# gMedAI-Lab/GAViKO

Hardware: AMD Instinct MI355X
Metric: MRI volumes/sec (fwd+bwd) ViT-B/16 gaviko, 120x160x160 (higher is better)
Workload: dtype bf16

## Files before the change

### gaviko_amd/csrc/gemm8p_bf16.hip

```cpp
#include "gemm_epilogue.hpp"

namespace gvk {

namespace {
constexpr int kUnit = 128 * 128;
constexpr int kBuf = 4 * kUnit;
constexpr int kLds = 2 * kBuf;

#define GVK_VMCNT(n) __builtin_amdgcn_s_waitcnt(0x0F70 | ((n) & 0xF) | (((n) >> 4) << 14))
#define GVK_LGKMCNT0() __builtin_amdgcn_s_waitcnt(0xC07F)

#ifdef GVK_STAMPS
#define GVK_STAMP(k) st_[k] = __builtin_amdgcn_s_memtime();
#ifndef GVK_ABLATE
#define GVK_ABLATE 0
#endif
#else
#define GVK_STAMP(k)
#define GVK_ABLATE 0
#endif
}

template <int EPI, int VAR>
__global__ __launch_bounds__(512) void gemm8p_kernel(GemmArgs p) {
  constexpr int BM = 256, BN = 256, BK = 64;
  extern __shared__ __attribute__((aligned(16))) char smem[];

  const int nwg = p.nbm * p.nbn;
  int wg;
  {
    const int bid = blockIdx.x, xcd = bid & 7, q = nwg >> 3, r = nwg & 7;
    wg = (xcd < r ? xcd * (q + 1) : r * (q + 1) + (xcd - r) * q) + (bid >> 3);
  }
  constexpr int GROUP_M = 8;
  const int gsz = GROUP_M * p.nbn;
  const int grp = wg / gsz, first_m = grp * GROUP_M;
  const int gm = min(p.nbm - first_m, GROUP_M);
  const int rem = wg - grp * gsz;
  const int tile_m = first_m + rem % gm, tile_n = rem / gm;
  const int m0 = tile_m * BM, n0 = tile_n * BN;

  const int lane = lane_id();
  const int wave = wave_id();
  const int wr = wave >> 2, wc = wave & 3;
#ifdef GVK_STAMPS
  unsigned long long st_[32];
#pragma unroll
  for (int k = 0; k < 32; ++k) st_[k] = 0;
  GVK_STAMP(0)
  const unsigned long long rt0_ = __builtin_amdgcn_s_memrealtime();
#endif
  const int l15 = lane & 15, lq = lane >> 4;

  const bf16* __restrict__ Ag = p.A + (size_t)m0 * p.lda;
  const bf16* __restrict__ Wg = p.W + (size_t)n0 * p.ldw;
  int aoff[2][2], woff[2][2];
#pragma unroll
  for (int r = 0; r < 2; ++r) {
    const int lr = (r * 8 + wave) * 8 + (lane >> 3), slot = lane & 7;
#pragma unroll
    for (int h = 0; h < 2; ++h) {
      const int mrow = min(128 * (lr >> 6) + 64 * h + (lr & 63), p.a_rows - 1 - m0);
      aoff[h][r] = mrow * p.lda + ((slot ^ swz_a128(lr)) << 3);
      const int nrow = 64 * (lr >> 5) + 32 * h + (lr & 31);
      woff[h][r] = nrow * p.ldw + ((slot ^ swz_w(lr)) << 3);
    }
  }
#define GVK_STAGE(U, T)                                                                                      \
  {                                                                                                          \
    const int t_ = (T);                                                                                      \
    char* dst_ = smem + (t_ & 1) * kBuf + (U) * kUnit + wave * 1024;                                         \
    const int k0_ = t_ * BK;                                                                                 \
    if constexpr ((U) == 0 || (U) == 2) {                                                                    \
      glds16(Wg + woff[(U) >> 1][0] + k0_, dst_);                                                            \
      glds16(Wg + woff[(U) >> 1][1] + k0_, dst_ + 8192);                                                     \
    } else {                                                                                                 \
      glds16(Ag + aoff[(U) >> 1][0] + k0_, dst_);                                                            \
      glds16(Ag + aoff[(U) >> 1][1] + k0_, dst_ + 8192);                                                     \
    }                                                                                                        \
  }

#define GVK_STAGE_HALF(U, T, R)                                                                              \
  if constexpr ((GVK_ABLATE & 1) == 0) {                                                                     \
    const int t_ = (T);                                                                                      \
    char* dst_ = smem + (t_ & 1) * kBuf + (U) * kUnit + wave * 1024 + (R) * 8192;                            \
    if constexpr ((U) == 0 || (U) == 2) glds16(Wg + woff[(U) >> 1][R] + t_ * BK, dst_);                      \
    else glds16(Ag + aoff[(U) >> 1][R] + t_ * BK, dst_);                                                     \
  }

  int ra[2], rw[2];
  {
    const int arow = 64 * wr + l15, wrow = 32 * wc + 8 * (l15 >> 2) + (l15 & 3);
#pragma unroll
    for (int ks = 0; ks < 2; ++ks) {
      ra[ks] = arow * 128 + (((4 * ks + lq) ^ swz_a128(arow)) << 4);
      rw[ks] = wrow * 128 + (((4 * ks + lq) ^ swz_w(wrow)) << 4);
    }
  }
  bf16x8 xa[4][2], w0[2][2], w1[2][2];
#define GVK_READ_A(MQ, BASE)                                                                                 \
  if constexpr ((GVK_ABLATE & 4) == 0)                                                                       \
  _Pragma("unroll") for (int i = 0; i < 4; ++i)                                                              \
  _Pragma("unroll") for (int ks = 0; ks < 2; ++ks)                                                           \
      xa[i][ks] = *(const bf16x8*)((BASE) + ((MQ) ? 3 : 1) * kUnit + ra[ks] + i * 2048);
#define GVK_READ_W(NQ, WREG, BASE)                                                                           \
  if constexpr ((GVK_ABLATE & 4) == 0)                                                                       \
  _Pragma("unroll") for (int j = 0; j < 2; ++j)                                                              \
  _Pragma("unroll") for (int ks = 0; ks < 2; ++ks)                                                           \
      WREG[j][ks] = *(const bf16x8*)((BASE) + ((NQ) ? 2 : 0) * kUnit + rw[ks] + j * 512);

  f32x4 acc[8][4];
#pragma unroll
  for (int i = 0; i < 8; ++i)
#pragma unroll
    for (int j = 0; j < 4; ++j) acc[i][j] = f32x4{0.f, 0.f, 0.f, 0.f};
#define GVK_MMA4(MQ, NQ, WREG, C_)                                                                           \
  if constexpr ((GVK_ABLATE & 2) == 0)                                                                       \
  _Pragma("unroll") for (int i = 2 * ((C_) & 1); i < 2 * ((C_) & 1) + 2; ++i)                                \
  _Pragma("unroll") for (int j = 0; j < 2; ++j)                                                              \
      acc[4 * (MQ) + i][2 * (NQ) + j] =                                                                      \
          __builtin_amdgcn_mfma_f32_16x16x32_bf16(WREG[j][(C_) >> 1], xa[i][(C_) >> 1], acc[4 * (MQ) + i][2 * (NQ) + j], 0, 0, 0);

#define GVK_COMPUTE(MQ, NQ, WREG, DO_STAGE, SU, ST_, SB)                                                     \
  __builtin_amdgcn_sched_barrier(0);                                                                         \
  __builtin_amdgcn_s_barrier();                                                                              \
  if constexpr ((SB) >= 0) { GVK_STAMP((SB) < 0 ? 0 : (SB)) }                                                \
  GVK_LGKMCNT0();                                                                                            \
  if constexpr ((SB) >= 0) { GVK_STAMP((SB) < 0 ? 0 : (SB) + 1) }                                            \
  __builtin_amdgcn_sched_barrier(0);                                                                         \
  __builtin_amdgcn_s_setprio(1);                                                                             \
  GVK_MMA4(MQ, NQ, WREG, 0)                                                                                  \
  if constexpr (VAR == 1 && (DO_STAGE)) {                                                                    \
    __builtin_amdgcn_sched_barrier(0);                                                                       \
    GVK_STAGE_HALF(SU, ST_, 0)                                                                               \
    __builtin_amdgcn_sched_barrier(0);                                                                       \
  }                                                                                                          \
  GVK_MMA4(MQ, NQ, WREG, 1)                                                                                  \
  GVK_MMA4(MQ, NQ, WREG, 2)                                                                                  \
  if constexpr (VAR == 1 && (DO_STAGE)) {                                                                    \
    __builtin_amdgcn_sched_barrier(0);                                                                       \
    GVK_STAGE_HALF(SU, ST_, 1)                                                                               \
    __builtin_amdgcn_sched_barrier(0);                                                                       \
  }                                                                                                          \
  GVK_MMA4(MQ, NQ, WREG, 3)                                                                                  \
  __builtin_amdgcn_s_setprio(0);                                                                             \
  __builtin_amdgcn_sched_barrier(0);                                                                         \
  if constexpr ((SB) >= 0) { GVK_STAMP((SB) < 0 ? 0 : (SB) + 2) }                                            \
  __builtin_amdgcn_s_barrier();                                                                              \
  if constexpr ((SB) >= 0) { GVK_STAMP((SB) < 0 ? 0 : (SB) + 3) }                                            \
  __builtin_amdgcn_sched_barrier(0);

#define GVK_KTILE(T, ST, VM0, VM1, VM3, SB)                                                                      \
  {                                                                                                          \
    const int tt_ = (T);                                                                                     \
    const char* base_ = smem + (tt_ & 1) * kBuf;                                                             \
    GVK_READ_W(0, w0, base_)                                                                                 \
    GVK_READ_A(0, base_)                                                                                     \
    if constexpr (VAR == 0 && ((ST) & 1) != 0 && (GVK_ABLATE & 1) == 0) GVK_STAGE(2, tt_ + 1)                                         \
    GVK_VMCNT(VM0);                                                                                          \
    GVK_COMPUTE(0, 0, w0, ((ST) & 1) != 0, 3, tt_ + 1, SB)                                                       \
    GVK_READ_W(1, w1, base_)                                                                                 \
    if constexpr (VAR == 0 && ((ST) & 2) != 0 && (GVK_ABLATE & 1) == 0) GVK_STAGE(3, tt_ + 1)                                         \
    GVK_VMCNT(VM1);                                                                                          \
    GVK_COMPUTE(0, 1, w1, ((ST) & 2) != 0, 0, tt_ + 2, (SB) < 0 ? -1 : (SB) + 4)                                                       \
    GVK_READ_A(1, base_)                                                                                     \
    if constexpr (VAR == 0 && ((ST) & 4) != 0 && (GVK_ABLATE & 1) == 0) GVK_STAGE(0, tt_ + 2)                                         \
    GVK_COMPUTE(1, 1, w1, ((ST) & 4) != 0, 1, tt_ + 2, (SB) < 0 ? -1 : (SB) + 8)                                                       \
    if constexpr (VAR == 0 && ((ST) & 8) != 0 && (GVK_ABLATE & 1) == 0) GVK_STAGE(1, tt_ + 2)                                         \
    GVK_VMCNT(VM3);                                                                                          \
    GVK_COMPUTE(1, 0, w0, ((ST) & 8) != 0, 2, tt_ + 2, (SB) < 0 ? -1 : (SB) + 12)                                                       \
  }

  const int nt = p.K / BK;
  GVK_STAGE(0, 0) GVK_STAGE(1, 0) GVK_STAGE(2, 0) GVK_STAGE(3, 0)
  GVK_STAGE(0, 1) GVK_STAGE(1, 1)
  if constexpr (VAR == 1) {
    GVK_STAGE(2, 1)
    GVK_VMCNT(10);
  } else {
    GVK_VMCNT(8);
  }
  __builtin_amdgcn_s_barrier();
  if (wr == 1) __builtin_amdgcn_s_barrier();
  __builtin_amdgcn_sched_barrier(0);
  GVK_STAMP(1)
  int t = 0;
#ifdef GVK_STAMPS
  for (; t < nt - 3; ++t) GVK_KTILE(t, 15, 8, 8, 8, -1)
  GVK_STAMP(2)
  if (nt >= 3) { GVK_KTILE(t, 15, 8, 8, 8, 4) ++t; }
  GVK_STAMP(20)
#else
  for (; t < nt - 2; ++t) GVK_KTILE(t, 15, 8, 8, 8, -1)
#endif
  if constexpr (VAR == 1) {
    GVK_KTILE(t, 1, 8, 8, 4, -1)
    ++t;
    GVK_KTILE(t, 0, 2, 0, 63, -1)
  } else {
    GVK_KTILE(t, 3, 8, 8, 4, -1)
    ++t;
    GVK_KTILE(t, 0, 2, 0, 63, -1)
  }
  if (wr == 0) __builtin_amdgcn_s_barrier();
#undef GVK_KTILE
#undef GVK_COMPUTE
#undef GVK_MMA4
#undef GVK_STAGE_HALF
#undef GVK_READ_A
#undef GVK_READ_W
#undef GVK_STAGE

  GVK_STAMP(21)
#ifdef GVK_STAMPS
  if constexpr ((GVK_ABLATE & 2) != 0) {
#pragma unroll
    for (int i = 0; i < 4; ++i) { asm volatile("" ::"v"(xa[i][0]), "v"(xa[i][1])); }
    asm volatile("" ::"v"(w0[0][0]), "v"(w0[1][1]), "v"(w1[0][0]), "v"(w1[1][1]));
  }
  const bf16* aux_keep = p.aux;
  p.aux = nullptr;
#endif
  gemm_epilogue<EPI, false, 8, 4>(p, acc, m0 + 128 * wr, n0 + 64 * wc, l15, lq);
#ifdef GVK_STAMPS
  __builtin_amdgcn_s_waitcnt(0x0F70);
  GVK_STAMP(22)
  st_[23] = rt0_;
  st_[24] = __builtin_amdgcn_s_memrealtime();
  if (aux_keep != nullptr && lane == 0) {
    unsigned long long* o = (unsigned long long*)aux_keep + ((size_t)blockIdx.x * 8 + wave) * 32;
#pragma unroll
    for (int k = 0; k < 32; ++k) o[k] = st_[k];
  }
#endif
}

template <int EPI, int VAR>
static int launch8p(const GemmArgs& a, hipStream_t stream) {
  static bool attr_set = false;
  if (!attr_set) {
    hipError_t e = hipFuncSetAttribute(reinterpret_cast<const void*>(&gemm8p_kernel<EPI, VAR>), hipFuncAttributeMaxDynamicSharedMemorySize, kLds);
    if (e != hipSuccess) return set_error(-3, "hipFuncSetAttribute(gemm8p): %s", hipGetErrorString(e));
    attr_set = true;
  }
  GemmArgs p = a;
  p.nbm = (a.M + 255) / 256;
  p.nbn = a.N / 256;
  p.a_rows = (a.M + 127) / 128 * 128;
  GVK_LAUNCH((gemm8p_kernel<EPI, VAR>), dim3(p.nbm * p.nbn), dim3(512), kLds, stream, p);
  return check_launch("gemm8p_bf16");
}

bool gemm8p_supports(int epilogue) {
  switch (epilogue) {
    case GVK_EPI_STORE_BF16: case GVK_EPI_BIAS_GELU_BF16: case GVK_EPI_GELU_BWD_BF16: case GVK_EPI_STORE_F32: case GVK_EPI_BIAS_RES_F32:
      return true;
    default:
      return false;
  }
}

template <int VAR>
static int launch8p_var(const GemmArgs& a, int epilogue, hipStream_t stream) {
  if (a.N % 256 != 0 || a.K % 64 != 0 || a.K < 128 || a.drop_thresh != 0u)
    return set_error(-2, "gemm8p: needs N %% 256 == 0, K %% 64 == 0, K >= 128 and no dropout (N=%d K=%d)", a.N, a.K);
  switch (epilogue) {
    case GVK_EPI_STORE_BF16: return launch8p<GVK_EPI_STORE_BF16, VAR>(a, stream);
    case GVK_EPI_BIAS_GELU_BF16: return launch8p<GVK_EPI_BIAS_GELU_BF16, VAR>(a, stream);
    case GVK_EPI_GELU_BWD_BF16: return launch8p<GVK_EPI_GELU_BWD_BF16, VAR>(a, stream);
    case GVK_EPI_STORE_F32: return launch8p<GVK_EPI_STORE_F32, VAR>(a, stream);
    case GVK_EPI_BIAS_RES_F32: return launch8p<GVK_EPI_BIAS_RES_F32, VAR>(a, stream);
    default: return set_error(-2, "gemm8p: epilogue %d is not built on the 256x256 eight-phase kernel", epilogue);
  }
}

int launch_gemm8p(const GemmArgs& a, int epilogue, int variant, hipStream_t stream) {
  return variant == 0 ? launch8p_var<0>(a, epilogue, stream) : launch8p_var<1>(a, epilogue, stream);
}

}
```

### gaviko_amd/csrc/gemm_bf16.hip

```cpp
#include "gemm_epilogue.hpp"

namespace gvk {

template <int BK>
__device__ __forceinline__ int swz_chunk(int row) {
  if constexpr (BK == 64) return (row >> 1) & 7;
  else return (0x78 >> (((row >> 2) & 3) * 2)) & 3;
}

template <int BM, int BN, int EPI, int BK = 64, bool DROP = false, int NS = 2, int NW = 4, bool SPLITK = false>
__global__ __launch_bounds__(64 * NW) void gemm_nt_kernel(GemmArgs p) {
  static_assert(NW == 4 || NW == 8, "4 or 8 waves");
  static_assert(!SPLITK || (NW == 4 && !DROP), "split-K is built on the 4-wave loops");
  static_assert(BK == 64, "the interleaved weight-row mapping is built for 128-byte tile rows");
  static_assert(NS >= 2 && NS <= 4, "2..4 LDS stages");
  constexpr int WM = BM / (NW / 2), WN = BN / 2;
  constexpr int MT = WM / 16, NT = WN / 16;
  constexpr int ROWB = BK * 2;
  constexpr int RPI = 1024 / ROWB;
  constexpr int CPR = ROWB / 16;
  constexpr int A_BYTES = BM * ROWB, W_BYTES = BN * ROWB, STAGE = A_BYTES + W_BYTES;
  extern __shared__ __attribute__((aligned(16))) char smem[];

  const int nwg = p.nbm * p.nbn;
  int wg;
  [[maybe_unused]] int piece = 0;
  if constexpr (SPLITK) {
    const int nu = nwg * p.ksplit;
    const int bid = blockIdx.x, xcd = bid & 7, q = nu >> 3, r = nu & 7;
    const int u = (xcd < r ? xcd * (q + 1) : r * (q + 1) + (xcd - r) * q) + (bid >> 3);
    wg = u / p.ksplit;
    piece = u - wg * p.ksplit;
  } else {
    const int bid = blockIdx.x, xcd = bid & 7, q = nwg >> 3, r = nwg & 7;
    wg = (xcd < r ? xcd * (q + 1) : r * (q + 1) + (xcd - r) * q) + (bid >> 3);
  }
  const int GROUP_M = p.group_m;
  const int gsz = GROUP_M * p.nbn;
  const int grp = wg / gsz, first_m = grp * GROUP_M;
  const int gm = min(p.nbm - first_m, GROUP_M);
  const int rem = wg - grp * gsz;
  int tile_m = first_m + rem % gm, tile_n = rem / gm;
  if (p.xcd_panels > 0) {
    tile_m = wg / p.nbn;
    tile_n = wg - tile_m * p.nbn;
  }
  const int m0 = tile_m * p.m_stride, n0 = tile_n * BN;

  const int lane = lane_id();
  const int wave = wave_id();
  const int wm = wave >> 1, wn = wave & 1;
  const int l15 = lane & 15, lq = lane >> 4;

  const bf16* __restrict__ Ag = p.A + (size_t)m0 * p.lda;
  const bf16* __restrict__ Wg = p.W + (size_t)n0 * p.ldw;
  if constexpr (SPLITK) {
    Ag += (size_t)piece * p.kt_per * BK;
    Wg += (size_t)piece * p.kt_per * BK;
  }

  auto stage = [&](int buf, int kt) {
    char* sA = smem + buf * STAGE;
    char* sW = sA + A_BYTES;
    const int k0 = kt * BK;
    const int rsub = lane / CPR, slot = lane % CPR;
#pragma unroll
    for (int r = 0; r < BM / (NW * RPI); ++r) {
      const int row = (r * NW + wave) * RPI + rsub;
      const int chunk = slot ^ swz_chunk<BK>(row);
      int srow = row;
      if constexpr (BM > 128 || 128 % BM != 0) srow = min(row, p.a_rows - 1 - m0);
      glds16(Ag + (size_t)srow * p.lda + k0 + chunk * 8, sA + (r * NW + wave) * 1024);
    }
#pragma unroll
    for (int r = 0; r < BN / (NW * RPI); ++r) {
      const int row = (r * NW + wave) * RPI + rsub;
      const int chunk = slot ^ swz_w(row);
      glds16(Wg + (size_t)row * p.ldw + k0 + chunk * 8, sW + (r * NW + wave) * 1024);
    }
  };

  f32x4 acc[MT][NT];
#pragma unroll
  for (int i = 0; i < MT; ++i)
#pragma unroll
    for (int j = 0; j < NT; ++j) acc[i][j] = f32x4{0.f, 0.f, 0.f, 0.f};

  int nt = p.K / BK;
  if constexpr (SPLITK) nt = min(p.kt_per, nt - piece * p.kt_per);
  if constexpr (BK == 64) {
#define GVK_LOAD_FRAGS(SA, SW, KS, XA, WB)                                                                  \
  {                                                                                                         \
    const int chunk_ = (KS) * 4 + lq;                                                                       \
    _Pragma("unroll") for (int i = 0; i < MT; ++i) {                                                        \
      const int row = wm * WM + i * 16 + l15;                                                               \
      XA[i] = *(const bf16x8*)((SA) + row * ROWB + ((chunk_ ^ swz_chunk<BK>(row)) << 4));                   \
    }                                                                                                       \
    _Pragma("unroll") for (int j = 0; j < NT; ++j) {                                                        \
      const int row = wn * WN + 32 * (j >> 1) + 8 * (l15 >> 2) + 4 * (j & 1) + (l15 & 3);                   \
      WB[j] = *(const bf16x8*)((SW) + row * ROWB + ((chunk_ ^ swz_w(row)) << 4));                           \
    }                                                                                                       \
  }
#define GVK_MMA(XA, WB)                                                                                      \
  _Pragma("unroll") for (int i = 0; i < MT; ++i)                                                            \
  _Pragma("unroll") for (int j = 0; j < NT; ++j)                                                            \
      acc[i][j] = __builtin_amdgcn_mfma_f32_16x16x32_bf16(WB[j], XA[i], acc[i][j], 0, 0, 0);
    bf16x8 xa0[MT], wb0[NT], xa1[MT], wb1[NT];
    constexpr int PER_TILE = BM / (NW * RPI) + BN / (NW * RPI);
    if constexpr (NS == 2) {
    stage(0, 0);
    if (nt > 1) stage(1, 1);
    if (nt > 1) __builtin_amdgcn_s_waitcnt(0x0F70 | (PER_TILE & 0xF) | ((PER_TILE >> 4) << 14));
    else __builtin_amdgcn_s_waitcnt(0x0F70);
    __builtin_amdgcn_s_barrier();
    GVK_LOAD_FRAGS(smem, smem + A_BYTES, 0, xa0, wb0)
    __builtin_amdgcn_s_waitcnt(0xC07F);
#define GVK_TILE(T, PREFETCH)                                                                               \
    {                                                                                                       \
      const int buf = (T) & 1;                                                                              \
      const char* sA = smem + buf * STAGE;                                                                  \
      const char* sW = sA + A_BYTES;                                                                        \
      GVK_LOAD_FRAGS(sA, sW, 1, xa1, wb1)                                                                   \
      __builtin_amdgcn_sched_barrier(0);                                                                    \
      GVK_MMA(xa0, wb0)                                                                                     \
      __builtin_amdgcn_sched_barrier(0);                                                                    \
      __syncthreads();     \
      if (PREFETCH) stage(buf, (T) + 2);                                                                    \
      GVK_LOAD_FRAGS(smem + (buf ^ 1) * STAGE, smem + (buf ^ 1) * STAGE + A_BYTES, 0, xa0, wb0)             \
      __builtin_amdgcn_sched_barrier(0);                                                                    \
      GVK_MMA(xa1, wb1)                                                                                     \
      __builtin_amdgcn_sched_barrier(0);                                                                    \
      __builtin_amdgcn_s_waitcnt(0xC07F);     \
    }
    int t = 0;
    for (; t < nt - 2; ++t) GVK_TILE(t, true)
    for (; t < nt; ++t) GVK_TILE(t, false)
#undef GVK_TILE
    } else {
    static_assert((NS - 1) * PER_TILE <= 63, "vmcnt is a 6-bit counter");
#pragma unroll
    for (int sgi = 0; sgi < NS; ++sgi)
      if (sgi < nt) stage(sgi, sgi);
    {
      const int ahead = min(nt, NS) - 1;
      if (ahead >= 3) __builtin_amdgcn_s_waitcnt(0x0F70 | ((3 * PER_TILE) & 0xF) | (((3 * PER_TILE) >> 4) << 14));
      else if (ahead == 2) __builtin_amdgcn_s_waitcnt(0x0F70 | ((2 * PER_TILE) & 0xF) | (((2 * PER_TILE) >> 4) << 14));
      else if (ahead == 1) __builtin_amdgcn_s_waitcnt(0x0F70 | (PER_TILE & 0xF) | ((PER_TILE >> 4) << 14));
      else __builtin_amdgcn_s_waitcnt(0x0F70);
    }
    __builtin_amdgcn_s_barrier();
    GVK_LOAD_FRAGS(smem, smem + A_BYTES, 0, xa0, wb0)
    __builtin_amdgcn_s_waitcnt(0xC07F);
#define GVK_TILE3(T, BUF, PREFETCH, AHEAD, LAST)                                                            \
    {                                                                                                       \
      const int buf = (BUF);                                                                                \
      const int nxt = buf == NS - 1 ? 0 : buf + 1;                                                          \
      const char* sA = smem + buf * STAGE;                                                                  \
      const char* sW = sA + A_BYTES;                                                                        \
      GVK_LOAD_FRAGS(sA, sW, 1, xa1, wb1)                                                                   \
      __builtin_amdgcn_sched_barrier(0);                                                                    \
      GVK_MMA(xa0, wb0)                                                                                     \
      __builtin_amdgcn_sched_barrier(0);                                                                    \
       \
      __builtin_amdgcn_s_waitcnt(0x0070 | (((AHEAD) * PER_TILE) & 0xF) | ((((AHEAD) * PER_TILE) >> 4) << 14)); \
      __builtin_amdgcn_s_barrier();                                                                         \
      if (PREFETCH) stage(buf, (T) + NS);                                                                   \
      if (!(LAST)) GVK_LOAD_FRAGS(smem + nxt * STAGE, smem + nxt * STAGE + A_BYTES, 0, xa0, wb0)            \
      __builtin_amdgcn_sched_barrier(0);                                                                    \
      GVK_MMA(xa1, wb1)                                                                                     \
      __builtin_amdgcn_sched_barrier(0);                                                                    \
      __builtin_amdgcn_s_waitcnt(0xC07F);                                                                   \
    }
    int t = 0, b = 0;
    for (; t < nt - NS; ++t) {
      GVK_TILE3(t, b, true, NS - 2, false)
      b = b == NS - 1 ? 0 : b + 1;
    }
    for (; t < nt; ++t) {
      const int r = nt - 1 - t;
      if (NS > 3 && r == 3) GVK_TILE3(t, b, false, 2, false)
      else if (r == 2) GVK_TILE3(t, b, false, 1, false)
      else if (r == 1) GVK_TILE3(t, b, false, 0, false)
      else GVK_TILE3(t, b, false, 0, true)
      b = b == NS - 1 ? 0 : b + 1;
    }
#undef GVK_TILE3
    }
#undef GVK_LOAD_FRAGS
#undef GVK_MMA
  }

  if constexpr (SPLITK) {
    const int tile_id = tile_m * p.nbn + tile_n;
    constexpr int kPiece = NW * MT * NT * 64 * 4;
    float* const base = p.sk_part + ((size_t)tile_id * p.ksplit) * kPiece;
    const __amdgpu_buffer_rsrc_t rs = __builtin_amdgcn_make_buffer_rsrc((void*)base, 0, p.ksplit * kPiece * 4, 0x00020000);
    const int off = ((wave * MT * NT) * 64 + lane) * 16;
#pragma unroll
    for (int i = 0; i < MT; ++i)
#pragma unroll
      for (int j = 0; j < NT; ++j)
        __builtin_amdgcn_raw_buffer_store_b128(__builtin_bit_cast(u32x4, acc[i][j]), rs, (piece * kPiece) * 4 + off + (i * NT + j) * 1024, 0, 16);
    int* const s_last = (int*)smem;
    asm volatile("s_waitcnt vmcnt(0)" ::: "memory");
    __syncthreads();
    if (threadIdx.x == 0) {
      const int t = __hip_atomic_fetch_add(p.sk_tick + tile_id, 1, __ATOMIC_RELAXED, __HIP_MEMORY_SCOPE_AGENT);
      const int last = (t == p.ksplit - 1) ? 1 : 0;
      if (last) {
        __builtin_amdgcn_fence(__ATOMIC_ACQUIRE, "agent");
        asm volatile("s_waitcnt vmcnt(0)" ::: "memory");
        __hip_atomic_store(p.sk_tick + tile_id, 0, __ATOMIC_RELAXED, __HIP_MEMORY_SCOPE_AGENT);
      }
      *s_last = last;
    }
    __syncthreads();
    if (!*s_last) return;
    if (p.ksplit == 2) {
      const int pc = piece ^ 1;
#pragma unroll
      for (int i = 0; i < MT; ++i)
#pragma unroll
        for (int j = 0; j < NT; ++j) acc[i][j] += *(const f32x4*)((const char*)base + (size_t)pc * kPiece * 4 + off + (i * NT + j) * 1024);
    } else {
#pragma unroll
      for (int i = 0; i < MT; ++i)
#pragma unroll
        for (int j = 0; j < NT; ++j) acc[i][j] = f32x4{0.f, 0.f, 0.f, 0.f};
      for (int pc = 0; pc < p.ksplit; ++pc) {
#pragma unroll
        for (int i = 0; i < MT; ++i)
#pragma unroll
          for (int j = 0; j < NT; ++j) acc[i][j] += *(const f32x4*)((const char*)base + (size_t)pc * kPiece * 4 + off + (i * NT + j) * 1024);
      }
    }
  }
  gemm_epilogue<EPI, DROP, MT, NT>(p, acc, m0 + wm * WM, n0 + wn * WN, l15, lq);
}

template <int BM, int BN, int EPI, bool DROP = false, int NS = 2, int NW = 4, bool SPLITK = false>
static int launch_gemm(const GemmArgs& a, hipStream_t stream) {
  constexpr int BK = 64;
  constexpr int lds = NS * (BM + BN) * BK * 2;
  static bool attr_set = false;
  if (!attr_set) {
    hipError_t e = hipFuncSetAttribute(reinterpret_cast<const void*>(&gemm_nt_kernel<BM, BN, EPI, BK, DROP, NS, NW, SPLITK>),
                                       hipFuncAttributeMaxDynamicSharedMemorySize, lds);
    if (e != hipSuccess) return set_error(-3, "hipFuncSetAttribute(gemm %dx%d): %s", BM, BN, hipGetErrorString(e));
    attr_set = true;
  }
  GemmArgs p = a;
  p.nbm = (a.M + BM - 1) / BM;
  p.nbn = a.N / BN;
  p.a_rows = (a.M + 127) / 128 * 128;
  p.m_stride = BM;
  if (a.m_stride > 0) {
    if (a.m_stride < BM || (long)(a.nbm - 1) * a.m_stride + BM > p.a_rows)
      return set_error(-2, "gvk_gemm_nt_bf16: %d row panels of %d rows at stride %d do not fit %d (padded) rows", a.nbm, BM, a.m_stride, p.a_rows);
    p.nbm = a.nbm;
    p.m_stride = a.m_stride;
  }
  {
    const int per_xcd = (p.nbm * p.nbn) >> 3;
    int g = (per_xcd + p.nbn / 2) / p.nbn;
    g = g < 1 ? 1 : g > 8 ? 8 : g;
    static const int force = diag_env("GAVIKO_HIP_GEMM_GROUP_M") ? atoi(diag_env("GAVIKO_HIP_GEMM_GROUP_M")) : 0;
    p.group_m = force > 0 ? force : g;
  }
  const int grid = p.nbm * p.nbn;
  p.xcd_panels = 0;
  {
    static const int mode = diag_env("GAVIKO_HIP_GEMM_XCD_PANELS") ? atoi(diag_env("GAVIKO_HIP_GEMM_XCD_PANELS")) : 1;
    if (mode != 0 && NS >= 3 && grid <= 256) p.xcd_panels = 1;
  }
  if constexpr (SPLITK) {
    const int nt = a.K / BK;
    int s = 256 / (grid > 0 ? grid : 1);
    s = s < 1 ? 1 : s > 8 ? 8 : s;
    if (a.ksplit > 0) s = a.ksplit;
    if (s > nt / 2) s = nt / 2 > 0 ? nt / 2 : 1;
    p.kt_per = (nt + s - 1) / s;
    p.ksplit = (nt + p.kt_per - 1) / p.kt_per;
    constexpr size_t kPiece = (size_t)NW * (BM / (NW / 2) / 16) * (BN / 2 / 16) * 64 * 4 * 4;
    const size_t need = 1024 + (size_t)grid * p.ksplit * kPiece;
    if (a.sk_part == nullptr || a.sk_bytes < need || grid > 256)
      return set_error(-2, "gvk_gemm_nt_bf16: split-K workspace of %zu bytes needed (%zu given; at most 256 tiles)", need, a.sk_bytes);
    p.sk_tick = (int*)a.sk_part;
    p.sk_part = (float*)((char*)a.sk_part + 1024);
    GVK_LAUNCH((gemm_nt_kernel<BM, BN, EPI, BK, DROP, NS, NW, SPLITK>), dim3(grid * p.ksplit), dim3(64 * NW), lds, stream, p);
    return check_launch("gemm_nt_bf16 (split-K panels)");
  }
  GVK_LAUNCH((gemm_nt_kernel<BM, BN, EPI, BK, DROP, NS, NW, SPLITK>), dim3(grid), dim3(64 * NW), lds, stream, p);
  return check_launch("gemm_nt_bf16");
}

static long wide_lo() {
  static const long v = diag_env("GAVIKO_HIP_GEMM_WIDE_LO") ? atol(diag_env("GAVIKO_HIP_GEMM_WIDE_LO")) : 140;
  return v;
}

template <int EPI>
static int dispatch_tile(const GemmArgs& a, int tile, hipStream_t stream) {
  if (a.m_stride > 0) {
    if (tile == 0) tile = (a.N % 128 == 0 && a.drop_thresh == 0u) ? 4064128 : 64064;
    if (tile == 8256256 || tile == 7256256 || tile == 256256) return set_error(-2, "gvk_gemm_nt_bf16: strided row panels run on the 4-wave tiles only");
  }
  if (tile == 0) {
    const int bn = (a.N % 128 == 0) ? 128 : 64;
    const long t128 = (long)((a.M + 127) / 128) * (a.N / bn);
    static const int n768 = diag_env("GAVIKO_HIP_GEMM_N768") ? atoi(diag_env("GAVIKO_HIP_GEMM_N768")) : 3128;
    const int bm = (t128 >= 384) ? 128 : 64;
    tile = bm * 1000 + bn;
    if constexpr (EPI == GVK_EPI_STORE_BF16 || EPI == GVK_EPI_BIAS_GELU_BF16 || EPI == GVK_EPI_GELU_BWD_BF16) {
      static const int wide = diag_env("GAVIKO_HIP_GEMM_WIDE") ? atoi(diag_env("GAVIKO_HIP_GEMM_WIDE")) : 8;
      const long t256 = (long)((a.M + 255) / 256) * (a.N / 256);
      static const bool wide_bwd = diag_env("GAVIKO_HIP_GEMM_WIDE_BWD") == nullptr || diag_env("GAVIKO_HIP_GEMM_WIDE_BWD")[0] != '0';
      if (wide != 0 && a.N % 256 == 0 && a.drop_thresh == 0u && t256 >= wide_lo() && t256 <= 256 && (EPI != GVK_EPI_GELU_BWD_BF16 || wide_bwd))
        tile = (wide == 256 || a.K < 128) ? 256256 : 8256256;
    }
    static const long t64_hi = diag_env("GAVIKO_HIP_GEMM_T64HI") ? atol(diag_env("GAVIKO_HIP_GEMM_T64HI")) : 130;
    if (bm == 64 && bn == 128 && t128 <= 256 && a.K >= 512 && a.drop_thresh == 0u) {
      if (n768 == 3128) {
        long best = -1; int best_bm = 128;
        for (int cand : {128, 96, 64}) {
          const long tiles = (long)((a.M + cand - 1) / cand) * (a.N / 128);
          const long cost = ((tiles + 255) / 256) * (cand + 128);
          if (best < 0 || cost < best) { best = cost; best_bm = cand; }
        }
        static const int force_bm = diag_env("GAVIKO_HIP_GEMM_BM") ? atoi(diag_env("GAVIKO_HIP_GEMM_BM")) : 0;
        if (force_bm == 128 || force_bm == 96 || force_bm == 64) best_bm = force_bm;
        else if (t128 <= t64_hi && best_bm == 128) best_bm = 64;
        tile = best_bm == 64 ? 3064128 : best_bm == 96 ? 3096128 : 3128128;
      }
      else if (n768 == 128) tile = 128128;
      else if (n768 == 3064) tile = 3064128;
    }
  }
  if (a.drop_thresh != 0u) {
    if constexpr (EPI == GVK_EPI_BIAS_RES_F32 || EPI == GVK_EPI_BIAS_GELU_BF16 || EPI == GVK_EPI_GELU_BWD_BF16) {
      switch (tile) {
        case 128128: return launch_gemm<128, 128, EPI, true>(a, stream);
        case 128064: return launch_gemm<128, 64, EPI, true>(a, stream);
        case 64128: return launch_gemm<64, 128, EPI, true>(a, stream);
        case 64064: return launch_gemm<64, 64, EPI, true>(a, stream);
        default: return set_error(-2, "gvk_gemm_nt_bf16: unsupported tile %d", tile);
      }
    } else {
      return set_error(-2, "gvk_gemm_nt_bf16: drop_p > 0 is supported by BIAS_RES_F32, BIAS_GELU_BF16 and GELU_BWD_BF16 only");
    }
  }
  switch (tile) {
    case 8256256: return launch_gemm8p(a, EPI, 0, stream);
    case 7256256: return launch_gemm8p(a, EPI, 1, stream);
    case 2128128:
      if (a.sk_part == nullptr) return set_error(-2, "gvk_gemm_nt_bf16: tile 2128128 needs splitk_ws");
      return launch_gemm<128, 128, EPI, false, 2, 4, true>(a, stream);
    case 3128128: return launch_gemm<128, 128, EPI, false, 3>(a, stream);
    case 3064128: return launch_gemm<64, 128, EPI, false, 3>(a, stream);
    case 4064128:
      if (a.sk_part != nullptr) return launch_gemm<64, 128, EPI, false, 4, 4, true>(a, stream);
      return launch_gemm<64, 128, EPI, false, 4>(a, stream);
    case 3096128: return launch_gemm<96, 128, EPI, false, 3>(a, stream);
    case 256256:
      if constexpr (EPI == GVK_EPI_STORE_BF16 || EPI == GVK_EPI_BIAS_GELU_BF16 || EPI == GVK_EPI_GELU_BWD_BF16) return launch_gemm<256, 256, EPI, false, 2, 8>(a, stream);
      else return set_error(-2, "gvk_gemm_nt_bf16: the 256x256 tile is built for STORE_BF16, BIAS_GELU_BF16 and GELU_BWD_BF16");
    case 128128: return launch_gemm<128, 128, EPI>(a, stream);
    case 128064: return launch_gemm<128, 64, EPI>(a, stream);
    case 64128: return launch_gemm<64, 128, EPI>(a, stream);
    case 64064: return launch_gemm<64, 64, EPI>(a, stream);
    default: return set_error(-2, "gvk_gemm_nt_bf16: unsupported tile %d", tile);
  }
}

}

extern "C" int gvk_gemm_stat_parts(int N) { return N / 64; }

extern "C" int gvk_gemm_nt_bf16(const gvk_gemm_desc* d, void* stream) {
  using namespace gvk;
  GVK_REQUIRE(d != nullptr, "gvk_gemm_nt_bf16: null descriptor");
  GVK_REQUIRE(d->a && d->w && d->M > 0 && d->N > 0 && d->K > 0, "gvk_gemm_nt_bf16: null operand or empty shape");
  GVK_REQUIRE(d->K % 64 == 0, "gvk_gemm_nt_bf16: K=%d must be a multiple of 64", d->K);
  GVK_REQUIRE(d->N % 64 == 0, "gvk_gemm_nt_bf16: N=%d must be a multiple of 64", d->N);
  GVK_REQUIRE(d->lda >= d->K && d->ldw >= d->K && d->lda % 8 == 0 && d->ldw % 8 == 0,
              "gvk_gemm_nt_bf16: lda/ldw must be >= K and multiples of 8");
  GVK_REQUIRE(d->ldo % 8 == 0 && d->ldo >= d->N, "gvk_gemm_nt_bf16: ldo=%d must be >= N and a multiple of 8 (16-byte row pieces)", d->ldo);
  if (d->tile != 0) {
    const int bn = d->tile % 1000;
    GVK_REQUIRE(d->tile < 1000000 || d->K % 32 == 0, "gvk_gemm_nt_bf16: K not a multiple of 32");
    GVK_REQUIRE(bn > 0 && d->N % bn == 0, "gvk_gemm_nt_bf16: N=%d not a multiple of the tile's BN", d->N);
  }
  GemmArgs a{};
  a.A = (const bf16*)d->a; a.W = (const bf16*)d->w; a.out0 = d->out0; a.out1 = d->out1;
  a.bias = d->bias; a.res = d->res; a.aux = (const bf16*)d->aux; a.pos = d->pos;
  a.M = d->M; a.N = d->N; a.K = d->K; a.lda = d->lda; a.ldw = d->ldw; a.ldo = d->ldo;
  a.ldres = d->ldres; a.ldaux = d->ldaux; a.rows_in = d->rows_in; a.rows_out = d->rows_out; a.row_off = d->row_off;
  GVK_REQUIRE(d->drop_p >= 0.f && d->drop_p < 1.f && (d->drop_p == 0.f || d->seed_ptr != nullptr), "gvk_gemm_nt_bf16: drop_p in [0,1) and a seed word");
  a.seed = d->seed; a.seed_ptr = (const unsigned long long*)d->seed_ptr; a.drop_thresh = drop_threshold_u32(d->drop_p);
  a.inv_keep = d->drop_p > 0.f ? 1.f / (1.f - d->drop_p) : 1.f;
  GVK_REQUIRE(d->scale_cols == 0 || (d->epilogue == GVK_EPI_STORE_BF16 && d->scale_cols > 0 && d->scale_cols % 8 == 0 && d->scale_cols <= d->N),
              "gvk_gemm_nt_bf16: scale_cols=%d needs the STORE_BF16 epilogue, a multiple of 8 and <= N", d->scale_cols);
  a.scale_cols = d->scale_cols; a.col_scale = d->col_scale;
  GVK_REQUIRE(d->ln_mean == nullptr || (d->epilogue == GVK_EPI_STORE_BF16 && d->ln_rstd && d->ln_c1 && d->bias),
              "gvk_gemm_nt_bf16: the LayerNorm fold needs the STORE_BF16 epilogue, ln_rstd, ln_c1 and bias (= sum_c beta[c] W[n][c])");
  a.ln_mean = d->ln_mean; a.ln_rstd = d->ln_rstd; a.ln_c1 = d->ln_c1;
  GVK_REQUIRE(d->stat_part == nullptr || (d->epilogue == GVK_EPI_BIAS_RES_F32_BF16 && d->N % 128 == 0 && (d->tile == 0 || d->tile % 1000 == 128)),
              "gvk_gemm_nt_bf16: stat_part needs the BIAS_RES_F32_BF16 epilogue on 128-column tiles (64-column groups)");
  a.stat_part = d->stat_part; a.stat_pivot = d->stat_pivot;
  GVK_REQUIRE((d->m_panels == 0 && d->m_stride == 0) || (d->m_panels > 0 && d->m_stride > 0 && d->epilogue != GVK_EPI_PATCH_F32),
              "gvk_gemm_nt_bf16: m_panels=%d / m_stride=%d: both positive (or both 0), not with the PATCH epilogue", d->m_panels, d->m_stride);
  a.m_stride = d->m_stride; a.nbm = d->m_panels;
  GVK_REQUIRE(d->splitk_ws == nullptr || ((d->m_panels > 0 || d->tile == 2128128) && ((uintptr_t)d->splitk_ws & 255) == 0),
              "gvk_gemm_nt_bf16: splitk_ws goes with strided row panels or tile 2128128 (256-byte aligned)");
  GVK_REQUIRE(d->ksplit >= 0 && d->ksplit <= 8 && (d->ksplit == 0 || d->splitk_ws != nullptr), "gvk_gemm_nt_bf16: ksplit=%d: 0 (auto) .. 8, with splitk_ws", d->ksplit);
  a.sk_part = (float*)d->splitk_ws; a.sk_bytes = d->splitk_ws_bytes; a.ksplit = d->ksplit;
  GVK_REQUIRE(d->aux_is_grad == 0 || (d->drop_p == 0.f && ((d->epilogue == GVK_EPI_BIAS_GELU_BF16 && d->out0) || d->epilogue == GVK_EPI_GELU_BWD_BF16)),
              "gvk_gemm_nt_bf16: aux_is_grad goes with BIAS_GELU_BF16 (out0 set) / GELU_BWD_BF16 and no dropout");
  a.aux_grad = d->aux_is_grad;
  hipStream_t s = (hipStream_t)stream;
  switch (d->epilogue) {
    case GVK_EPI_STORE_BF16:
      GVK_REQUIRE(d->out0, "gemm STORE_BF16: out0 null");
      return dispatch_tile<GVK_EPI_STORE_BF16>(a, d->tile, s);
    case GVK_EPI_BIAS_RES_F32:
      GVK_REQUIRE(d->out0 && d->res && d->ldres >= d->N && d->ldres % 4 == 0, "gemm BIAS_RES_F32: out0/res");
      return dispatch_tile<GVK_EPI_BIAS_RES_F32>(a, d->tile, s);
    case GVK_EPI_BIAS_RES_F32_BF16:
      GVK_REQUIRE(d->out0 && d->out1 && d->res && d->ldres >= d->N && d->ldres % 4 == 0, "gemm BIAS_RES_F32_BF16: out0/out1/res");
      return dispatch_tile<GVK_EPI_BIAS_RES_F32_BF16>(a, d->tile, s);
    case GVK_EPI_BIAS_GELU_BF16:
      GVK_REQUIRE(d->out1, "gemm BIAS_GELU_BF16: out1 null");
      return dispatch_tile<GVK_EPI_BIAS_GELU_BF16>(a, d->tile, s);
    case GVK_EPI_PATCH_F32:
      GVK_REQUIRE(d->out0 && d->pos && d->rows_in > 0 && d->rows_out >= d->rows_in + d->row_off && d->ldo == d->N,
                  "gemm PATCH_F32: out0/pos/rows_in/rows_out/row_off inconsistent (ldo must equal N)");
      return dispatch_tile<GVK_EPI_PATCH_F32>(a, d->tile, s);
    case GVK_EPI_GELU_BWD_BF16:
      GVK_REQUIRE(d->out0 && d->aux && d->ldaux >= d->N && d->ldaux % 8 == 0, "gemm GELU_BWD_BF16: out0/aux");
      return dispatch_tile<GVK_EPI_GELU_BWD_BF16>(a, d->tile, s);
    case GVK_EPI_STORE_F32:
      GVK_REQUIRE(d->out0, "gemm STORE_F32: out0 null");
      return dispatch_tile<GVK_EPI_STORE_F32>(a, d->tile, s);
    case GVK_EPI_BIAS_RELU_BF16:
      GVK_REQUIRE(d->out0, "gemm BIAS_RELU_BF16: out0 null");
      return dispatch_tile<GVK_EPI_BIAS_RELU_BF16>(a, d->tile, s);
    case GVK_EPI_RELU_BWD_BF16:
      GVK_REQUIRE(d->out0 && d->aux && d->ldaux >= d->N && d->ldaux % 8 == 0, "gemm RELU_BWD_BF16: out0/aux");
      return dispatch_tile<GVK_EPI_RELU_BWD_BF16>(a, d->tile, s);
    default:
      return set_error(-2, "gvk_gemm_nt_bf16: unknown epilogue %d", d->epilogue);
  }
}
```

### gaviko_amd/csrc/gemm_epilogue.hpp

```cpp
#pragma once
#include "common.hpp"
#include "dropout.hpp"
#include "../../include/gaviko_hip.h"

namespace gvk {

struct GemmArgs {
  const bf16* A;
  const bf16* W;
  void* out0;
  void* out1;
  const float* bias;
  const float* res;
  const bf16* aux;
  const float* pos;
  int M, N, K, lda, ldw, ldo, ldres, ldaux;
  int rows_in, rows_out, row_off;
  int nbm, nbn;
  int group_m;
  int xcd_panels;
  int a_rows;
  int m_stride;
  int ksplit, kt_per;
  float* sk_part;
  int* sk_tick;
  size_t sk_bytes;
  unsigned long long seed; const unsigned long long* seed_ptr; unsigned int drop_thresh; float inv_keep;
  int scale_cols; float col_scale;
  const float* ln_mean; const float* ln_rstd; const float* ln_c1;
  float* stat_part;
  const float* stat_pivot;
  int aux_grad;
};

__device__ __forceinline__ int swz_a128(int row) { return (row >> 1) & 7; }
__device__ __forceinline__ int swz_w(int row) { return ((row >> 1) & 1) | (((row >> 3) & 3) << 1); }

template <int EPI, bool DROP, int MT, int NT>
__device__ __forceinline__ void gemm_epilogue(const GemmArgs& p, f32x4 (&acc)[MT][NT], const int mbase, const int nbase, const int l15, const int lq) {
  static_assert(NT % 2 == 0, "tile pairs");
  constexpr int NP = NT / 2;
  constexpr bool kRes = EPI == GVK_EPI_BIAS_RES_F32 || EPI == GVK_EPI_BIAS_RES_F32_BF16;
  constexpr bool kAux = EPI == GVK_EPI_GELU_BWD_BF16 || EPI == GVK_EPI_RELU_BWD_BF16;
  constexpr bool kPos = EPI == GVK_EPI_PATCH_F32;
  constexpr bool kFold = EPI == GVK_EPI_STORE_BF16;
  constexpr bool kStat = EPI == GVK_EPI_BIAS_RES_F32_BF16;
  f32x4 bv[NP][2];
  [[maybe_unused]] f32x4 c1v[NP][2];
#pragma unroll
  for (int jp = 0; jp < NP; ++jp) {
    bv[jp][0] = bv[jp][1] = f32x4{0.f, 0.f, 0.f, 0.f};
    const int n = nbase + 32 * jp + 8 * lq;
    if (p.bias != nullptr) {
      bv[jp][0] = *(const f32x4*)(p.bias + n);
      bv[jp][1] = *(const f32x4*)(p.bias + n + 4);
    }
    if constexpr (kFold) {
      c1v[jp][0] = c1v[jp][1] = f32x4{0.f, 0.f, 0.f, 0.f};
      if (p.ln_mean != nullptr) {
        c1v[jp][0] = *(const f32x4*)(p.ln_c1 + n);
        c1v[jp][1] = *(const f32x4*)(p.ln_c1 + n + 4);
      }
    }
  }
  struct Side { f32x4 r0[NP], r1[NP]; bf16x8 a8[NP]; float mu, rs, pv; };
  auto fetch = [&](const int i, Side& sd) {
    const int m = mbase + i * 16 + l15;
    if (m >= p.M) return;
    if constexpr (kFold) {
      if (p.ln_mean != nullptr) { sd.mu = p.ln_mean[m]; sd.rs = p.ln_rstd[m]; }
    }
    if constexpr (kStat) sd.pv = p.stat_pivot != nullptr ? p.stat_pivot[m] : 0.f;
#pragma unroll
    for (int jp = 0; jp < NP; ++jp) {
      const int n = nbase + 32 * jp + 8 * lq;
      if constexpr (kRes) {
        const float* rp = p.res + (size_t)m * p.ldres + n;
        sd.r0[jp] = *(const f32x4*)rp;
        sd.r1[jp] = *(const f32x4*)(rp + 4);
      } else if constexpr (kPos) {
        const float* pp = p.pos + (size_t)(m % p.rows_in) * p.N + n;
        sd.r0[jp] = *(const f32x4*)pp;
        sd.r1[jp] = *(const f32x4*)(pp + 4);
      } else if constexpr (kAux) {
        sd.a8[jp] = *(const bf16x8*)(p.aux + (size_t)m * p.ldaux + n);
      }
    }
  };
  Side cur, nxt;
  fetch(0, cur);
#pragma unroll
  for (int i = 0; i < MT; ++i) {
    if (i + 1 < MT) fetch(i + 1, nxt);
    const int m = mbase + i * 16 + l15;
    [[maybe_unused]] float ps1 = 0.f, ps2 = 0.f;
    if (m < p.M) {
      size_t orow = (size_t)m;
      if constexpr (kPos) {
        const int s = m / p.rows_in;
        orow = (size_t)s * p.rows_out + p.row_off + (m - s * p.rows_in);
      }
#pragma unroll
      for (int jp = 0; jp < NP; ++jp) {
        const int n = nbase + 32 * jp + 8 * lq;
        float v[8];
#pragma unroll
        for (int e = 0; e < 4; ++e) { v[e] = acc[i][2 * jp][e] + bv[jp][0][e]; v[4 + e] = acc[i][2 * jp + 1][e] + bv[jp][1][e]; }
        if constexpr (kFold) {
          if (p.ln_mean != nullptr) {
#pragma unroll
            for (int e = 0; e < 4; ++e) {
              v[e] = __builtin_fmaf(__builtin_fmaf(-cur.mu, c1v[jp][0][e], acc[i][2 * jp][e]), cur.rs, bv[jp][0][e]);
              v[4 + e] = __builtin_fmaf(__builtin_fmaf(-cur.mu, c1v[jp][1][e], acc[i][2 * jp + 1][e]), cur.rs, bv[jp][1][e]);
            }
          }
        }
        auto store_f32 = [&](float* dst) {
          *(f32x4*)dst = f32x4{v[0], v[1], v[2], v[3]};
          *(f32x4*)(dst + 4) = f32x4{v[4], v[5], v[6], v[7]};
        };
        auto store_bf16 = [&](bf16* dst) {
          bf16x8 o;
#pragma unroll
          for (int e = 0; e < 8; ++e) o[e] = (bf16)v[e];
          *(bf16x8*)dst = o;
        };
        [[maybe_unused]] auto drop8 = [&]() {
          const unsigned long long sd = p.seed + *p.seed_ptr;
#pragma unroll
          for (int e = 0; e < 8; ++e) v[e] *= drop_scale(sd, (unsigned long long)m * p.N + n + e, p.drop_thresh, p.inv_keep);
        };
        if constexpr (EPI == GVK_EPI_STORE_BF16) {
          if (n < p.scale_cols) {
#pragma unroll
            for (int e = 0; e < 8; ++e) v[e] *= p.col_scale;
          }
          store_bf16((bf16*)p.out0 + (size_t)m * p.ldo + n);
        } else if constexpr (kRes) {
          if constexpr (DROP) drop8();
#pragma unroll
          for (int e = 0; e < 4; ++e) { v[e] += cur.r0[jp][e]; v[4 + e] += cur.r1[jp][e]; }
          store_f32((float*)p.out0 + (size_t)m * p.ldo + n);
          if constexpr (EPI == GVK_EPI_BIAS_RES_F32_BF16) {
            store_bf16((bf16*)p.out1 + (size_t)m * p.ldo + n);
#pragma unroll
            for (int e = 0; e < 8; ++e) { const float dv = v[e] - cur.pv; ps1 += dv; ps2 = __builtin_fmaf(dv, dv, ps2); }
          }
        } else if constexpr (EPI == GVK_EPI_BIAS_GELU_BF16) {
          if (p.aux_grad != 0) {
            bf16x8 g8;
#pragma unroll
            for (int e = 0; e < 8; ++e) {
              float y, dy;
              gelu_fast_both(v[e], y, dy);
              v[e] = y;
              g8[e] = (bf16)dy;
            }
            *(bf16x8*)((bf16*)p.out0 + (size_t)m * p.ldo + n) = g8;
          } else {
            if (p.out0 != nullptr) store_bf16((bf16*)p.out0 + (size_t)m * p.ldo + n);
#pragma unroll
            for (int e = 0; e < 8; ++e) v[e] = gelu_fast(v[e]);
          }
          if constexpr (DROP) drop8();
          store_bf16((bf16*)p.out1 + (size_t)m * p.ldo + n);
        } else if constexpr (kPos) {
#pragma unroll
          for (int e = 0; e < 4; ++e) { v[e] += cur.r0[jp][e]; v[4 + e] += cur.r1[jp][e]; }
          store_f32((float*)p.out0 + orow * p.ldo + n);
          if (p.out1 != nullptr) store_f32((float*)p.out1 + (size_t)m * p.ldo + n);
        } else if constexpr (EPI == GVK_EPI_GELU_BWD_BF16) {
          if constexpr (DROP) drop8();
#pragma unroll
          for (int e = 0; e < 8; ++e) v[e] *= p.aux_grad != 0 ? (float)cur.a8[jp][e] : gelu_fast_grad((float)cur.a8[jp][e]);
          store_bf16((bf16*)p.out0 + (size_t)m * p.ldo + n);
        } else if constexpr (EPI == GVK_EPI_STORE_F32) {
          store_f32((float*)p.out0 + (size_t)m * p.ldo + n);
        } else if constexpr (EPI == GVK_EPI_BIAS_RELU_BF16) {
#pragma unroll
          for (int e = 0; e < 8; ++e) v[e] = fmaxf(v[e], 0.f);
          store_bf16((bf16*)p.out0 + (size_t)m * p.ldo + n);
        } else if constexpr (EPI == GVK_EPI_RELU_BWD_BF16) {
#pragma unroll
          for (int e = 0; e < 8; ++e) v[e] = (float)cur.a8[jp][e] > 0.f ? v[e] : 0.f;
          store_bf16((bf16*)p.out0 + (size_t)m * p.ldo + n);
        }
      }
    }
    if constexpr (kStat) {
      if (p.stat_part != nullptr) {
        ps1 += __shfl_xor(ps1, 16, 64); ps2 += __shfl_xor(ps2, 16, 64);
        ps1 += __shfl_xor(ps1, 32, 64); ps2 += __shfl_xor(ps2, 32, 64);
        if (lq == 0 && m < p.M) *(f32x2*)(p.stat_part + ((size_t)(nbase / (16 * NT)) * p.M + m) * 2) = f32x2{ps1, ps2};
      }
    }
    cur = nxt;
  }
}

int launch_gemm8p(const GemmArgs& a, int epilogue, int variant, hipStream_t stream);
bool gemm8p_supports(int epilogue);

}
```

Before: 771.3.

## Stage GEMM epilogue through LDS for row-contiguous coalesced stores

Adds a new epilogue that writes each 16-row accumulator group into a swizzled per-wave LDS slab, reusing the dead pipeline buffers. Lanes then re-read it so each lane owns contiguous columns of one row, and stores plus residual/aux loads become full-row coalesced vectors. The LayerNorm stat reduction is redone with DPP row shifts, and the bf16 side output is packed across lane pairs. It is enabled for all epilogues in both GEMM kernels, at the cost of extra LDS traffic and a more complex lane mapping that could hide indexing bugs.

Result: no change. 773.6 (median of 2 runs) (+0.3%).

```diff
diff --git a/gaviko_amd/csrc/gemm8p_bf16.hip b/gaviko_amd/csrc/gemm8p_bf16.hip
--- a/gaviko_amd/csrc/gemm8p_bf16.hip
+++ b/gaviko_amd/csrc/gemm8p_bf16.hip
@@ -221,7 +221,11 @@
   const bf16* aux_keep = p.aux;
   p.aux = nullptr;
 #endif
-  gemm_epilogue<EPI, false, 8, 4>(p, acc, m0 + 128 * wr, n0 + 64 * wc, l15, lq);
+  if constexpr (gemm_epi_rows<EPI>()) {
+    gemm_epilogue_rows<EPI, false, 8, 2>(p, acc, m0 + 128 * wr, n0 + 64 * wc, lane, smem + wave * 8192);
+  } else {
+    gemm_epilogue<EPI, false, 8, 4>(p, acc, m0 + 128 * wr, n0 + 64 * wc, l15, lq);
+  }
 #ifdef GVK_STAMPS
   __builtin_amdgcn_s_waitcnt(0x0F70);
   GVK_STAMP(22)
diff --git a/gaviko_amd/csrc/gemm_bf16.hip b/gaviko_amd/csrc/gemm_bf16.hip
--- a/gaviko_amd/csrc/gemm_bf16.hip
+++ b/gaviko_amd/csrc/gemm_bf16.hip
@@ -235,7 +235,17 @@
       }
     }
   }
-  gemm_epilogue<EPI, DROP, MT, NT>(p, acc, m0 + wm * WM, n0 + wn * WN, l15, lq);
+  if constexpr (NT == 4 && NW == 4 && gemm_epi_rows<EPI>()) {
+    constexpr int avail = SPLITK ? NS * STAGE - 1024 : NS == 2 ? STAGE : NS * STAGE;
+    constexpr int SLABS = avail >= NW * 8192 ? 2 : 1;
+    static_assert(avail >= NW * SLABS * 4096, "epilogue slabs fit the dead pipeline buffers");
+    char* epi = smem;
+    if constexpr (SPLITK) epi = smem + 1024;
+    else if constexpr (NS == 2) epi = smem + ((nt - 1) & 1) * STAGE;
+    gemm_epilogue_rows<EPI, DROP, MT, SLABS>(p, acc, m0 + wm * WM, n0 + wn * WN, lane, epi + wave * (SLABS * 4096));
+  } else {
+    gemm_epilogue<EPI, DROP, MT, NT>(p, acc, m0 + wm * WM, n0 + wn * WN, l15, lq);
+  }
 }
 
 template <int BM, int BN, int EPI, bool DROP = false, int NS = 2, int NW = 4, bool SPLITK = false>
diff --git a/gaviko_amd/csrc/gemm_epilogue.hpp b/gaviko_amd/csrc/gemm_epilogue.hpp
--- a/gaviko_amd/csrc/gemm_epilogue.hpp
+++ b/gaviko_amd/csrc/gemm_epilogue.hpp
@@ -198,6 +198,205 @@
   }
 }
 
+template <int EPI> constexpr bool gemm_epi_f32_stream() {
+  return EPI == GVK_EPI_BIAS_RES_F32 || EPI == GVK_EPI_BIAS_RES_F32_BF16 || EPI == GVK_EPI_PATCH_F32 || EPI == GVK_EPI_STORE_F32;
+}
+template <int EPI> constexpr bool gemm_epi_rows() { return true; }
+
+__device__ __forceinline__ float dpp_row_shr1(float x) { return __builtin_bit_cast(float, __builtin_amdgcn_update_dpp(0, __builtin_bit_cast(int, x), 0x111, 0xF, 0xF, true)); }
+__device__ __forceinline__ float dpp_row_shr7(float x) { return __builtin_bit_cast(float, __builtin_amdgcn_update_dpp(0, __builtin_bit_cast(int, x), 0x117, 0xF, 0xF, true)); }
+__device__ __forceinline__ float dpp_row_shl2(float x) { return __builtin_bit_cast(float, __builtin_amdgcn_update_dpp(0, __builtin_bit_cast(int, x), 0x102, 0xF, 0xF, true)); }
+__device__ __forceinline__ float dpp_row_shl4(float x) { return __builtin_bit_cast(float, __builtin_amdgcn_update_dpp(0, __builtin_bit_cast(int, x), 0x104, 0xF, 0xF, true)); }
+__device__ __forceinline__ unsigned dpp_swap1(unsigned x) { return (unsigned)__builtin_amdgcn_update_dpp(0, (int)x, 0xB1, 0xF, 0xF, true); }
+
+template <int EPI, bool DROP, int MT, int SLABS>
+__device__ __forceinline__ void gemm_epilogue_rows(const GemmArgs& p, f32x4 (&acc)[MT][4], const int mbase, const int nbase, const int lane, char* const slab) {
+  static_assert(SLABS == 1 || SLABS == 2, "one slab, or two so that group i+1 is written before group i is read");
+  constexpr bool kF32 = gemm_epi_f32_stream<EPI>();
+  constexpr int CPL = kF32 ? 4 : 8;
+  constexpr int LPR = 64 / CPL;
+  constexpr int RPP = 64 / LPR;
+  constexpr int NQ = 16 / RPP;
+  constexpr int CH = CPL / 4;
+  constexpr bool kRes = EPI == GVK_EPI_BIAS_RES_F32 || EPI == GVK_EPI_BIAS_RES_F32_BF16;
+  constexpr bool kAux = EPI == GVK_EPI_GELU_BWD_BF16 || EPI == GVK_EPI_RELU_BWD_BF16;
+  constexpr bool kPos = EPI == GVK_EPI_PATCH_F32;
+  constexpr bool kFold = EPI == GVK_EPI_STORE_BF16;
+  constexpr bool kStat = EPI == GVK_EPI_BIAS_RES_F32_BF16;
+  const int l15 = lane & 15, lq = lane >> 4;
+  const int lc = lane % LPR, lr = lane / LPR;
+  const int n = nbase + CPL * lc;
+  float bv[CPL];
+  [[maybe_unused]] float c1v[CPL];
+#pragma unroll
+  for (int c = 0; c < CH; ++c) {
+    f32x4 b = f32x4{0.f, 0.f, 0.f, 0.f}, c1 = f32x4{0.f, 0.f, 0.f, 0.f};
+    if (p.bias != nullptr) b = *(const f32x4*)(p.bias + n + 4 * c);
+    if constexpr (kFold) {
+      if (p.ln_mean != nullptr) c1 = *(const f32x4*)(p.ln_c1 + n + 4 * c);
+    }
+#pragma unroll
+    for (int e = 0; e < 4; ++e) {
+      bv[4 * c + e] = b[e];
+      if constexpr (kFold) c1v[4 * c + e] = c1[e];
+    }
+  }
+  struct Side { f32x4 r[NQ]; bf16x8 a8[NQ]; float mu[NQ], rs[NQ], pv[NQ]; };
+  auto fetch = [&](const int i, Side& sd) {
+#pragma unroll
+    for (int q = 0; q < NQ; ++q) {
+      const int m = mbase + i * 16 + q * RPP + lr;
+      if (m >= p.M) continue;
+      if constexpr (kFold) {
+        if (p.ln_mean != nullptr) { sd.mu[q] = p.ln_mean[m]; sd.rs[q] = p.ln_rstd[m]; }
+      }
+      if constexpr (kStat) sd.pv[q] = p.stat_pivot != nullptr ? p.stat_pivot[m] : 0.f;
+      if constexpr (kRes) sd.r[q] = *(const f32x4*)(p.res + (size_t)m * p.ldres + n);
+      else if constexpr (kPos) sd.r[q] = *(const f32x4*)(p.pos + (size_t)(m % p.rows_in) * p.N + n);
+      else if constexpr (kAux) sd.a8[q] = *(const bf16x8*)(p.aux + (size_t)m * p.ldaux + n);
+    }
+  };
+  auto put = [&](const int i) {
+    char* const s = slab + (SLABS == 2 ? (i & 1) * 4096 : 0) + l15 * 256;
+#pragma unroll
+    for (int j = 0; j < 4; ++j) *(f32x4*)(s + (((8 * (j >> 1) + 2 * lq + (j & 1)) ^ (l15 & 7)) << 4)) = acc[i][j];
+  };
+  Side cur, nxt;
+  fetch(0, cur);
+  if constexpr (SLABS == 2) put(0);
+#pragma unroll
+  for (int i = 0; i < MT; ++i) {
+    if (i + 1 < MT) fetch(i + 1, nxt);
+    if constexpr (SLABS == 2) { if (i + 1 < MT) put(i + 1); }
+    else put(i);
+    [[maybe_unused]] u32x2 pk[NQ];
+#pragma unroll
+    for (int q = 0; q < NQ; ++q) {
+      const int rr = q * RPP + lr;
+      const int m = mbase + i * 16 + rr;
+      float v[CPL];
+      {
+        const char* const s = slab + (SLABS == 2 ? (i & 1) * 4096 : 0) + rr * 256;
+#pragma unroll
+        for (int c = 0; c < CH; ++c) {
+          const f32x4 t = *(const f32x4*)(s + (((CH * lc + c) ^ (rr & 7)) << 4));
+#pragma unroll
+          for (int e = 0; e < 4; ++e) v[4 * c + e] = t[e];
+        }
+      }
+      if constexpr (kStat) pk[q] = u32x2{0u, 0u};
+      if (m < p.M) {
+        bool fold = false;
+        if constexpr (kFold) fold = p.ln_mean != nullptr;
+        if (fold) {
+          if constexpr (kFold) {
+#pragma unroll
+            for (int e = 0; e < CPL; ++e) v[e] = __builtin_fmaf(__builtin_fmaf(-cur.mu[q], c1v[e], v[e]), cur.rs[q], bv[e]);
+          }
+        } else {
+#pragma unroll
+          for (int e = 0; e < CPL; ++e) v[e] = v[e] + bv[e];
+        }
+        auto store_row = [&](void* base, const size_t row) {
+          if constexpr (kF32) {
+            *(f32x4*)((float*)base + row * p.ldo + n) = f32x4{v[0], v[1], v[2], v[3]};
+          } else {
+            bf16x8 o;
+#pragma unroll
+            for (int e = 0; e < CPL; ++e) o[e] = (bf16)v[e];
+            *(bf16x8*)((bf16*)base + row * p.ldo + n) = o;
+          }
+        };
+        [[maybe_unused]] auto drop = [&]() {
+          const unsigned long long sd = p.seed + *p.seed_ptr;
+#pragma unroll
+          for (int e = 0; e < CPL; ++e) v[e] *= drop_scale(sd, (unsigned long long)m * p.N + n + e, p.drop_thresh, p.inv_keep);
+        };
+        if constexpr (EPI == GVK_EPI_STORE_BF16) {
+          if (n < p.scale_cols) {
+#pragma unroll
+            for (int e = 0; e < CPL; ++e) v[e] *= p.col_scale;
+          }
+          store_row(p.out0, (size_t)m);
+        } else if constexpr (kRes) {
+          if constexpr (DROP) drop();
+#pragma unroll
+          for (int e = 0; e < 4; ++e) v[e] += cur.r[q][e];
+          store_row(p.out0, (size_t)m);
+          if constexpr (kStat) {
+            const bf16x4 o = bf16x4{(bf16)v[0], (bf16)v[1], (bf16)v[2], (bf16)v[3]};
+            pk[q] = __builtin_bit_cast(u32x2, o);
+            if (p.stat_part != nullptr) {
+              float s1 = 0.f, s2 = 0.f;
+#pragma unroll
+              for (int hop = 0; hop < 4; ++hop) {
+                if (hop == 1 || hop == 3) { s1 = dpp_row_shr1(s1); s2 = dpp_row_shr1(s2); }
+                if (hop == 2) { s1 = dpp_row_shr7(s1); s2 = dpp_row_shr7(s2); }
+#pragma unroll
+                for (int e = 0; e < 4; ++e) { const float dv = v[e] - cur.pv[q]; s1 += dv; s2 = __builtin_fmaf(dv, dv, s2); }
+              }
+              s1 += dpp_row_shl2(s1); s2 += dpp_row_shl2(s2);
+              s1 += dpp_row_shl4(s1); s2 += dpp_row_shl4(s2);
+              if (lc == 9) *(f32x2*)(p.stat_part + ((size_t)(nbase / 64) * p.M + m) * 2) = f32x2{s1, s2};
+            }
+          }
+        } else if constexpr (EPI == GVK_EPI_BIAS_GELU_BF16) {
+          if (p.aux_grad != 0) {
+            bf16x8 g8;
+#pragma unroll
+            for (int e = 0; e < CPL; ++e) {
+              float y, dy;
+              gelu_fast_both(v[e], y, dy);
+              v[e] = y;
+              g8[e] = (bf16)dy;
+            }
+            *(bf16x8*)((bf16*)p.out0 + (size_t)m * p.ldo + n) = g8;
+          } else {
+            if (p.out0 != nullptr) store_row(p.out0, (size_t)m);
+#pragma unroll
+            for (int e = 0; e < CPL; ++e) v[e] = gelu_fast(v[e]);
+          }
+          if constexpr (DROP) drop();
+          store_row(p.out1, (size_t)m);
+        } else if constexpr (kPos) {
+          const int s = m / p.rows_in;
+#pragma unroll
+          for (int e = 0; e < 4; ++e) v[e] += cur.r[q][e];
+          store_row(p.out0, (size_t)s * p.rows_out + p.row_off + (m - s * p.rows_in));
+          if (p.out1 != nullptr) store_row(p.out1, (size_t)m);
+        } else if constexpr (EPI == GVK_EPI_GELU_BWD_BF16) {
+          if constexpr (DROP) drop();
+#pragma unroll
+          for (int e = 0; e < CPL; ++e) v[e] *= p.aux_grad != 0 ? (float)cur.a8[q][e] : gelu_fast_grad((float)cur.a8[q][e]);
+          store_row(p.out0, (size_t)m);
+        } else if constexpr (EPI == GVK_EPI_STORE_F32) {
+          store_row(p.out0, (size_t)m);
+        } else if constexpr (EPI == GVK_EPI_BIAS_RELU_BF16) {
+#pragma unroll
+          for (int e = 0; e < CPL; ++e) v[e] = fmaxf(v[e], 0.f);
+          store_row(p.out0, (size_t)m);
+        } else if constexpr (EPI == GVK_EPI_RELU_BWD_BF16) {
+#pragma unroll
+          for (int e = 0; e < CPL; ++e) v[e] = (float)cur.a8[q][e] > 0.f ? v[e] : 0.f;
+          store_row(p.out0, (size_t)m);
+        }
+      }
+    }
+    if constexpr (kStat) {
+#pragma unroll
+      for (int q = 0; q < NQ; q += 2) {
+        const bool odd = (lc & 1) != 0;
+        const u32x2 give = odd ? pk[q] : pk[q + 1];
+        const u32x2 got = u32x2{dpp_swap1(give[0]), dpp_swap1(give[1])};
+        const u32x4 o = odd ? u32x4{got[0], got[1], pk[q + 1][0], pk[q + 1][1]} : u32x4{pk[q][0], pk[q][1], got[0], got[1]};
+        const int m = mbase + i * 16 + (q + (odd ? 1 : 0)) * RPP + lr;
+        if (m < p.M) *(u32x4*)((bf16*)p.out1 + (size_t)m * p.ldo + nbase + 8 * (lc >> 1)) = o;
+      }
+    }
+    cur = nxt;
+  }
+}
+
 int launch_gemm8p(const GemmArgs& a, int epilogue, int variant, hipStream_t stream);
 bool gemm8p_supports(int epilogue);
 
```
